# aerospaceresearch/DirectDemod

Measured on AMD Instinct MI355X. Metric: IQ MSamples/s through 255-tap FIR+FM demod, higher is better.
Workload: dtype f32; 1 GPU; C2: 2.4 MS/s complex64 IQ (u8 grid, FM tone + noise), offsetFreq 25 kHz NCO + 255-tap Hamming FIR + FM demod, single chunk, 2^26 samples per GPU, device resident; samples_per_gpu=67108864, ntaps=255, decimation=1, kernel=k_chain_cos1k

## Files before the change

### directdemod_amd/_hip.py

```python
import ctypes as C
import functools
import os
import threading
from fractions import Fraction

import numpy as np

_HERE = os.path.dirname(os.path.abspath(__file__))
LIB_PATH = os.path.join(_HERE, "libdirectdemod_hip.so")
if os.environ.get("DD_LIB_PATH"):
    LIB_PATH = os.path.abspath(os.environ["DD_LIB_PATH"])
    import sys as _sys
    _sys.stderr.write("directdemod_amd: DD_LIB_PATH set, loading %s instead of the product library\n" % LIB_PATH)

DD_OK = 0
DD_ERR_INVALID = -1
DD_ERR_HIP = -2
DD_ERR_NOMEM = -3
DD_ERR_UNSUPPORTED = -4
DD_ERR_NODEVICE = -5
DD_ERR_TIMEOUT = -6

DD_HIST_ZEROS, DD_HIST_ONES, DD_HIST_GIVEN = 0, 1, 2
DD_CHAIN_NCO, DD_CHAIN_FM, DD_CHAIN_U8_INPUT, DD_CHAIN_FORCE_DIRECT, DD_CHAIN_TIGHT = 1, 2, 4, 8, 16
# ... 11 lines not shown
class HipError(RuntimeError):
    pass


_p = C.c_void_p
_i64 = C.c_int64
_u64 = C.c_uint64
_int = C.c_int
_sz = C.c_size_t
_pp = C.POINTER(C.c_void_p)
_pi64 = C.POINTER(C.c_int64)

SIGNATURES = {
    "dd_last_error": (C.c_char_p, []),
    "dd_version": (C.c_char_p, []),
    "dd_device_count": (_int, [C.POINTER(_int)]),
    "dd_set_device": (_int, [_int]),
    "dd_get_device": (_int, [C.POINTER(_int)]),
    "dd_copy_warmup": (_int, []),
    "dd_code_warmup": (_int, []),
    "dd_device_name": (_int, [C.c_char_p, _int]),
    "dd_malloc": (_int, [_pp, _sz]),
    "dd_free": (_int, [_p]),
    "dd_memset": (_int, [_p, _int, _sz, _p]),
    "dd_host_alloc_pinned": (_int, [_pp, _sz]),
    "dd_host_free_pinned": (_int, [_p]),
    "dd_host_register": (_int, [_p, _sz]),
    "dd_host_unregister": (_int, [_p]),
    "dd_debug_fill_lds": (_int, [C.c_uint32, _p]),
    "dd_debug_select_kernel": (_int, [C.c_char_p]),
    "dd_debug_seam": (_int, [_int, _int]),
    "dd_debug_fft1k_plan": (_int, [_i64, _int, _int, _int, _int, C.POINTER(_int)]),
    "dd_debug_cos1k_plan": (_int, [_i64, _int, _int, _int, C.POINTER(_int)]),
    "dd_debug_decimw_plan": (_int, [_i64, _i64, _int, _int, _int, _int, C.POINTER(_i64)]),
    "dd_debug_decimb_lds_check": (_int, [_int, _int, _int, C.POINTER(_i64)]),
    "dd_debug_chain_select": (_int, [C.POINTER(C.c_double), _int, _int, _int, _int, C.c_char_p, C.POINTER(_int)]),
    "dd_debug_cos_fit": (_int, [C.POINTER(C.c_double), _int, C.POINTER(C.c_double), C.POINTER(_int)]),
    "dd_debug_sync_envelope": (_int, [_p, _i64, _int, _int, _p, _p]),
    "dd_memcpy_h2d": (_int, [_p, _p, _sz, _p]),
    "dd_memcpy_d2h": (_int, [_p, _p, _sz, _p]),
    "dd_memcpy_d2d": (_int, [_p, _p, _sz, _p]),
    "dd_stream_create": (_int, [_pp]),
    "dd_stream_destroy": (_int, [_p]),
    "dd_stream_sync": (_int, [_p]),
    "dd_event_create": (_int, [_pp]),
    "dd_event_destroy": (_int, [_p]),
    "dd_event_record": (_int, [_p, _p]),
    "dd_event_elapsed_ms": (_int, [_p, _p, C.POINTER(C.c_float)]),
    "dd_event_sync": (_int, [_p]),
    "dd_stream_wait_event": (_int, [_p, _p]),
    "dd_u8iq_to_c64": (_int, [_p, _p, _i64, _p]),
    "dd_nco_c64": (_int, [_p, _p, _i64, _u64, _i64, _p]),
    "dd_nco_c64_freqs": (_int, [_p, _p, _i64, _p, C.c_double, _i64, _p]),
    "dd_fir_create": (_int, [_pp, C.POINTER(C.c_double), _int]),
    "dd_fir_destroy": (_int, [_p]),
    "dd_fir_reset": (_int, [_p, _int, _p, _p]),
    "dd_fir_reset_hist_f64": (_int, [_p, C.POINTER(C.c_double), _p]),
    "dd_fir_c64": (_int, [_p, _p, _p, _i64, _int, _p]),
    "dd_fir_f64": (_int, [_p, _p, _p, _i64, _int, _p]),
    "dd_filtfilt_f64": (_int, [C.POINTER(C.c_double), _int, _p, _p, _i64, _int, _p]),
    "dd_filtfilt_c64": (_int, [C.POINTER(C.c_double), _int, _p, _p, _i64, _p]),
    "dd_iir_create": (_int, [_pp, C.POINTER(C.c_double), C.POINTER(C.c_double), _int, C.POINTER(C.c_double)]),
    "dd_iir_destroy": (_int, [_p]),
    "dd_iir_f64": (_int, [_p, _p, _p, _i64, _int, _int, _p]),
    "dd_iir_c64": (_int, [_p, _p, _p, _i64, _int, _p]),
    "dd_iir_filtfilt_f64": (_int, [_p, _p, _p, _i64, _int, _p]),
# ... 420 lines not shown
```

### directdemod_amd/csrc/dd_chain.hip

```cpp
#include "dd_chain_tile_kernels.h"
#include "dd_cosfir.h"
#include "dd_fftfir.h"
#include <stdlib.h>
#include <atomic>
#include <mutex>

enum { DD_KSEL_UNREAD = -1, DD_KSEL_AUTO = 0, DD_KSEL_AB = 1, DD_KSEL_FFT1K = 2, DD_KSEL_COS1K = 3, DD_KSEL_DECIMP = 4 };
static std::atomic<int> g_kernel_sel{DD_KSEL_UNREAD};
static int kernel_sel_parse(const char* name) {
    if (!name || !*name || strcmp(name, "auto") == 0) return DD_KSEL_AUTO;
    if (strcmp(name, "ab") == 0) return DD_KSEL_AB;
    if (strcmp(name, "fft1k") == 0) return DD_KSEL_FFT1K;
    if (strcmp(name, "cos1k") == 0) return DD_KSEL_COS1K;
    if (strcmp(name, "decimp") == 0) return DD_KSEL_DECIMP;
    return -2;
}
static int kernel_sel() {
    int c = g_kernel_sel.load(std::memory_order_relaxed);
    if (c == DD_KSEL_UNREAD) {
        c = kernel_sel_parse(getenv("DD_MFMA_KERNEL"));
        if (c < 0) c = DD_KSEL_AUTO;
        g_kernel_sel.store(c, std::memory_order_relaxed);
    }
    return c;
// ... 689 lines not shown
}

extern "C" int dd_chain_reset(dd_chain* c, void* stream) {
    DD_REQUIRE(c, "h");
    c->abs_index = 0;
    if (c->fm) dd_fm_reset(c->fm);
    return dd_fir_reset(c->fir, DD_HIST_ONES, nullptr, stream);
}

static inline int chain_off(const dd_chain* c) {
    return next_off(c->abs_index, 0, c->M);
}

extern "C" int64_t dd_chain_out_count(const dd_chain* c, int64_t n) {
    if (!c || n < 0) return -1;
    return dd_fused_out_count(c->fm, n, c->M, chain_off(c));
}

extern "C" int dd_chain_path(const dd_chain* c) {
    if (!c) return DD_ERR_INVALID;
    const int family = fir_select(c->fir, c->M, c->flags, nullptr);
    return (family == DD_FAMILY_COS1K || family == DD_FAMILY_FFT1K || family == DD_FAMILY_MFMA) ? 1 : 0;
}

extern "C" int dd_fir_last_kernel(const dd_fir* f) {
    if (!f) return DD_ERR_INVALID;
    return f->last_kernel;
}

extern "C" long long dd_fir_launch_count(const dd_fir* f) {
    return f ? f->launches : -1;
}

extern "C" int dd_chain_last_kernel(const dd_chain* c) {
    if (!c) return DD_ERR_INVALID;
    return c->fir->last_kernel;
}

extern "C" int dd_chain_process(dd_chain* c, const void* in, void* out, int64_t n, int64_t* n_out, void* stream) {
    DD_REQUIRE(c && n >= 0, "h/n");
    const DDFusedArgs a = fused_args(in, out, n, c->flags & DD_CHAIN_NCO, c->cyc, c->abs_index, c->M, chain_off(c), c->flags, 1);
    int rc = dd_fused_launch(c->fir, c->fm, a, n_out, dd_stream(stream));
    if (rc == DD_OK) c->abs_index += n;
    return rc;
}

extern "C" int dd_chain_process_chunks(dd_chain* c, const void* in, void* out, const int64_t* bounds_host, int nchunks,
                                       int64_t* n_out_host, void* stream) {
    DD_REQUIRE(c && bounds_host && nchunks >= 0, "arguments");
    const char* in0 = reinterpret_cast<const char*>(in) + (nchunks > 0 ? in_elem_size(c->flags) * (size_t)bounds_host[0] : 0);
    int64_t consumed = 0;
    const int rc = fused_chunks(c->fir, c->fm, in0, out, bounds_host, nchunks, c->flags & DD_CHAIN_NCO, c->cyc, c->abs_index, c->M, chain_off(c),
                                c->flags, n_out_host, &consumed, dd_stream(stream));
    c->abs_index += consumed;
    return rc;
}

extern "C" int dd_chain_seek(dd_chain* c, int64_t abs_index, void* stream) {
    DD_REQUIRE(c && abs_index >= 0, "arguments");
    c->abs_index = abs_index;
    if (c->fm) dd_fm_reset(c->fm);
    return dd_fir_reset(c->fir, abs_index == 0 ? DD_HIST_ONES : DD_HIST_ZEROS, nullptr, stream);
}

extern "C" int dd_chain_prime(dd_chain* c, const void* halo_in, int64_t n_halo, int64_t abs_index, void* stream) {
    DD_REQUIRE(c && n_halo >= 0 && abs_index >= 0, "arguments");
// ... 29 lines not shown
```

### directdemod_amd/csrc/dd_cosfir.h

```cpp
#pragma once
#include "dd_chain_kernels.h"

int dd_cos1k_supported(const double* taps, int K, int M, int flags);
int dd_cos1k_create(void** st, const double* taps, int K);
void dd_cos1k_destroy(void* st);
int dd_cos1k_launch(void* st, const DDChainParams& P, hipStream_t stream);
```

### directdemod_amd/csrc/dd_cosfir.hip

```cpp
#include "dd_chain_kernels.h"
#include "dd_cosfir.h"
#include "dd_cosfit.h"
#include "dd_atan.h"
#include <stdlib.h>

typedef float v2f __attribute__((ext_vector_type(2)));
typedef float v4f __attribute__((ext_vector_type(4)));

#define C1_K 255
#define C1_C1 9.996940573e-01f
#define C1_S1 2.473442728e-02f
#define C1_C2 9.987764162e-01f
#define C1_S2 4.945371992e-02f
#define C1_WC0 9.226918151e-01f
#define C1_WS0 3.855383436e-01f
#define C1_WC1 7.027203712e-01f
#define C1_WS1 7.114661481e-01f
#define C1_WC2 -1.236815966e-02f
#define C1_WS2 9.999235114e-01f
#define C1_WC3 -9.996940573e-01f
#define C1_WS3 -2.473442728e-02f
#define C1_ROW 1024
#define C1_GROUP_BYTES 144
#define C1_BUF_BYTES (64 * C1_GROUP_BYTES)
// ... 60 lines not shown
__device__ __forceinline__ v2f c1_bperm(int addr, v2f v) { return (v2f){c1_bperm(addr, v.x), c1_bperm(addr, v.y)}; }

struct C1St { v2f C, S, R; };

#define C1_ROW_SHR(n) (0x110 + (n))
template <int CTRL>
__device__ __forceinline__ float c1_add_dpp(float r) {
    static_assert(CTRL == 0x111 || CTRL == 0x112 || CTRL == 0x114 || CTRL == 0x118, "dpp control");
    if (CTRL == 0x111) asm("v_add_f32_dpp %0, %0, %0 row_shr:1 row_mask:0xf bank_mask:0xf bound_ctrl:1" : "+v"(r));
    if (CTRL == 0x112) asm("v_add_f32_dpp %0, %0, %0 row_shr:2 row_mask:0xf bank_mask:0xf bound_ctrl:1" : "+v"(r));
    if (CTRL == 0x114) asm("v_add_f32_dpp %0, %0, %0 row_shr:4 row_mask:0xf bank_mask:0xf bound_ctrl:1" : "+v"(r));
    if (CTRL == 0x118) asm("v_add_f32_dpp %0, %0, %0 row_shr:8 row_mask:0xf bank_mask:0xf bound_ctrl:1" : "+v"(r));
    return r;
}
template <int CTRL>
__device__ __forceinline__ void c1_scan_step(C1St& t, float wc, float ws) {
    const v2f Cs = (v2f){c1_dpp0<CTRL>(t.C.x), c1_dpp0<CTRL>(t.C.y)};
    const v2f Ss = (v2f){c1_dpp0<CTRL>(t.S.x), c1_dpp0<CTRL>(t.S.y)};
    t.R = (v2f){c1_add_dpp<CTRL>(t.R.x), c1_add_dpp<CTRL>(t.R.y)};
    t.C = c1_fma(wc, Cs, c1_fma(-ws, Ss, t.C));
    t.S = c1_fma(ws, Cs, c1_fma(wc, Ss, t.S));
}

struct C1Carry {
    C1St W;
    C1St V63;
    v2f y63;
    v2f prow;
    int64_t pend_S;
    int cur;
};

#define C1_NO_PEND ((int64_t)-4611686018427387904LL)
__device__ __forceinline__ void c1_flush_angles(const DDCos1kArgs& A, const char* img, int64_t S, int lane) {
    float* const o = reinterpret_cast<float*>(A.out) + (S - A.s) + 4 * lane;
    const int G = lane >> 2, sw = (G >> 1) & 3;
    v4f v[4];
#pragma unroll
    for (int g = 0; g < 4; ++g) v[g] = *reinterpret_cast<const v4f*>(img + 64 * (16 * g + G) + 16 * ((lane & 3) ^ sw));
#pragma unroll
    for (int g = 0; g < 4; ++g) {
        *reinterpret_cast<v4f*>(o + 256 * g) = v[g];
    }
}

__device__ __forceinline__ void c1_cx_read(const char* img, int lane, v4f (&v)[8]) {
    const char* const rd = img + (lane >> 3) * C1_GROUP_BYTES + 16 * (lane & 7);
#pragma unroll
    for (int j = 0; j < 8; ++j) v[j] = *reinterpret_cast<const v4f*>(rd + 8 * j * C1_GROUP_BYTES);
}
__device__ __forceinline__ void c1_cx_store(const DDCos1kArgs& A, int64_t S, int lane, const v4f (&v)[8]) {
    float2* const o = reinterpret_cast<float2*>(A.out) + S + 2 * lane;
#pragma unroll
    for (int j = 0; j < 8; ++j) __builtin_nontemporal_store(v[j], reinterpret_cast<v4f*>(o + 128 * j));
}

template <bool U8>
__device__ __forceinline__ void c1_issue_loads(const DDCos1kArgs& A, int64_t S, int lane, v4f (&xin)[8]) {
    if (U8) {
        const v4f* p = reinterpret_cast<const v4f*>(reinterpret_cast<const unsigned char*>(A.in) + 2 * (S + 16 * lane));
        xin[0] = __builtin_nontemporal_load(p);
        xin[1] = __builtin_nontemporal_load(p + 1);
    } else {
        const v4f* p = reinterpret_cast<const v4f*>(reinterpret_cast<const float2*>(A.in) + S + 2 * lane);
#pragma unroll
        for (int j = 0; j < 8; ++j) xin[j] = __builtin_nontemporal_load(p + 64 * j);
    }
}

template <bool NCO>
__device__ __forceinline__ v2f c1_row_phasor(const DDCos1kArgs& A, int64_t S, v2f ql) {
    if (!NCO) return (v2f){1.f, 0.f};
    const uint64_t phase64 = (uint64_t)(A.abs0 + S) * A.cyc;
    const uint32_t lo = __builtin_amdgcn_readfirstlane((uint32_t)(phase64 >> (64 - DD_NCO_TBITS - 32)));
#if defined(__HIP_DEVICE_COMPILE__)
    typedef const __attribute__((address_space(4))) float2* c1_const_f2;
    const uint32_t k = __builtin_amdgcn_readfirstlane((uint32_t)(phase64 >> (64 - DD_NCO_TBITS)));
    const float2 Tk = ((c1_const_f2)A.nco_tbl)[k];
#else
    const float2 Tk = make_float2(1.f, 0.f);
#endif
    const float theta = (float)lo * (6.283185307179586f * 5.684341886080802e-14f);
    const float t2 = theta * theta;
    const float cc = fmaf(-0.5f, t2, 1.0f), ss = theta * fmaf(-0.16666667f, t2, 1.0f);
    const v2f pr = (v2f){fmaf(Tk.x, cc, Tk.y * ss), fmaf(Tk.y, cc, -Tk.x * ss)};
    return c1_cmul(pr, ql);
}

template <bool U8, bool NCO, bool EDGE, bool CX>
__device__ __forceinline__ void c1_row(const DDCos1kArgs& A, const DDCos1kLane& lt, const int lane, char* const lds,
                                       const int64_t S, const bool emit, const bool prefetch_next,
                                       v4f (&xin)[8], v4f (&xnext)[8], const v2f ql, C1Carry& cr) {
    const float c = C1_C1, s = C1_S1;
    char* const cur = lds + cr.cur;
    char* const own = cur + lane * C1_GROUP_BYTES;
    v4f pv[8];
    const int64_t cx_pend = CX ? cr.pend_S : C1_NO_PEND;
    if (CX && cx_pend != C1_NO_PEND) { c1_cx_read(cur, lane, pv); cr.pend_S = C1_NO_PEND; }
    const char* const old = lane < 16 ? lds + (C1_BUF_BYTES - cr.cur) + (48 + lane) * C1_GROUP_BYTES : cur + (lane - 16) * C1_GROUP_BYTES;
    v2f xt[16];
    if (EDGE) {
#pragma unroll
        for (int i = 0; i < 16; ++i) {
            const int64_t n = S + 16 * lane + i;
            v2f v = (v2f){0.f, 0.f};
            if (n < 0) {
                const int64_t ti = n + (C1_K - 1);
                if (ti >= 0) v = c1_v2(A.tail_in[ti]);
            } else if (n < A.L) {
                float2 x;
                if (U8) {
                    const uchar2 u = reinterpret_cast<const uchar2*>(A.in)[n];
                    x = make_float2((float)u.x - 127.5f, (float)u.y - 127.5f);
                } else {
                    x = reinterpret_cast<const float2*>(A.in)[n];
                }
                if (NCO) x = dd_cmul(x, dd_phasor((uint64_t)(A.abs0 + n) * A.cyc, A.nco_tbl));
                v = c1_v2(x);
            }
            xt[i] = v;
        }
#pragma unroll
        for (int t = 0; t < 8; ++t) *reinterpret_cast<v4f*>(own + 16 * t) = (v4f){xt[2 * t].x, xt[2 * t].y, xt[2 * t + 1].x, xt[2 * t + 1].y};
    } else {
        const v2f prow = cr.prow;
// ... 28 lines not shown
            v2f pj[8];
            if (NCO) {
                pj[0] = prow;
                pj[1] = c1_cmul(prow, c1_v2(A.q1));
                pj[2] = c1_cmul(prow, c1_v2(A.q2));
                pj[3] = c1_cmul(pj[2], c1_v2(A.q1));
                pj[4] = c1_cmul(prow, c1_v2(A.q4));
                pj[5] = c1_cmul(pj[4], c1_v2(A.q1));
                pj[6] = c1_cmul(pj[4], c1_v2(A.q2));
                pj[7] = c1_cmul(pj[6], c1_v2(A.q1));
            }
            v2f pj1[8], t0[8], t1[8];
            if (NCO) {
                const v2f e1 = c1_v2(A.e1);
#pragma unroll
                for (int j = 0; j < 8; ++j) t0[j] = c1_mul_lo(pj[j], e1);
#pragma unroll
                for (int j = 0; j < 8; ++j) pj1[j] = c1_fma_hi(pj[j], e1, t0[j]);
#pragma unroll
                for (int j = 0; j < 8; ++j) { t0[j] = c1_mul_lo((v2f){xin[j].x, xin[j].y}, pj[j]); t1[j] = c1_mul_lo((v2f){xin[j].z, xin[j].w}, pj1[j]); }
            }
#pragma unroll
            for (int j = 0; j < 8; ++j) {
                v2f x0 = (v2f){xin[j].x, xin[j].y}, x1 = (v2f){xin[j].z, xin[j].w};
                if (NCO) {
                    x0 = c1_fma_hi(x0, pj[j], t0[j]);
                    x1 = c1_fma_hi(x1, pj1[j], t1[j]);
                }
                *reinterpret_cast<v4f*>(wr + 8 * j * C1_GROUP_BYTES) = (v4f){x0.x, x0.y, x1.x, x1.y};
            }
        }
    }
    if (prefetch_next) { c1_issue_loads<U8>(A, S + C1_ROW, lane, xnext); cr.prow = c1_row_phasor<NCO>(A, S + C1_ROW, ql); }
    if (CX) { if (cx_pend != C1_NO_PEND) c1_cx_store(A, cx_pend, lane, pv); }
    else if (cr.pend_S != C1_NO_PEND) { c1_flush_angles(A, lds + (C1_BUF_BYTES - cr.cur), cr.pend_S, lane); cr.pend_S = C1_NO_PEND; }
    if (!EDGE && !U8) {
#pragma unroll
        for (int t = 0; t < 8; ++t) {
            const v4f v = *reinterpret_cast<const v4f*>(own + 16 * t);
            xt[2 * t] = (v2f){v.x, v.y};
            xt[2 * t + 1] = (v2f){v.z, v.w};
        }
    }
    v2f d[16];
    d[0] = *reinterpret_cast<const v2f*>(old + 8);
#pragma unroll
    for (int t = 1; t < 8; ++t) {
        const v4f v = *reinterpret_cast<const v4f*>(old + 16 * t);
        d[2 * t - 1] = (v2f){v.x, v.y};
        d[2 * t] = (v2f){v.z, v.w};
    }
    d[15] = *reinterpret_cast<const v2f*>(lane == 15 ? cur : old + C1_GROUP_BYTES);
    C1St t;
    {
        static constexpr float CW[16] = {1.000000000e+00f, 9.996940573e-01f, 9.987764162e-01f, 9.972476384e-01f, 9.951086592e-01f, 9.923607874e-01f,
                                         9.890057045e-01f, 9.850454633e-01f, 9.804824871e-01f, 9.753195679e-01f, 9.695598648e-01f, 9.632069021e-01f,
                                         9.562645670e-01f, 9.487371075e-01f, 9.406291296e-01f, 9.319455943e-01f};
        static constexpr float SW[16] = {0.000000000e+00f, 2.473442728e-02f, 4.945371992e-02f, 7.414275255e-02f, 9.878641831e-02f, 1.233696381e-01f,
                                         1.478773698e-01f, 1.722946174e-01f, 1.966064405e-01f, 2.207979630e-01f, 2.448543824e-01f, 2.687609789e-01f,
                                         2.925031245e-01f, 3.160662917e-01f, 3.394360625e-01f, 3.625981373e-01f};
        v2f C0 = xt[15], C1 = CW[1] * xt[14], S0 = SW[2] * xt[13], S1 = SW[1] * xt[14], R0 = xt[15] + xt[13], R1 = xt[14];
        C0 = c1_fma(CW[2], xt[13], C0);
#pragma unroll
        for (int i = 12; i >= 0; --i) {
            const int m = 15 - i;
            if (i & 1) { C0 = c1_fma(CW[m], xt[i], C0); S0 = c1_fma(SW[m], xt[i], S0); R0 += xt[i]; }
// ... 108 lines not shown
            for (int g = 0; g < 4; ++g) {
                float worst = -1.0f;
#pragma unroll
                for (int k = 0; k < 4; ++k) worst = fmaxf(worst, fmaf(-0.41421356f, z[4 * g + k].x, fabsf(z[4 * g + k].y)));
                if (__builtin_amdgcn_ballot_w64(worst >= 0.f) == 0) {
#pragma unroll
                    for (int k = 0; k < 4; ++k) ang[4 * g + k] = dd_atan_small(z[4 * g + k].y, z[4 * g + k].x);
                } else {
#pragma unroll
                    for (int k = 0; k < 4; ++k) ang[4 * g + k] = dd_atan2_poly(z[4 * g + k].y, z[4 * g + k].x);
                }
            }
        }
    }
    if (EDGE) {
        float* const o = reinterpret_cast<float*>(A.out) + (S - A.s) + 16 * lane;
#pragma unroll
        for (int i = 0; i < 16; ++i) {
            const int64_t n = S + 16 * lane + i;
            if (n >= A.s && n < A.L) o[i] = ang[i];
        }
        return;
    }
    char* const img = cur;
    {
        const int sw = (lane >> 1) & 3;
#pragma unroll
        for (int t = 0; t < 4; ++t)
            *reinterpret_cast<v4f*>(img + 64 * lane + 16 * (t ^ sw)) = (v4f){ang[4 * t], ang[4 * t + 1], ang[4 * t + 2], ang[4 * t + 3]};
    }
    cr.pend_S = S;
}

template <bool U8>
__device__ __forceinline__ void c1_prime_issue(const DDCos1kArgs& A, int64_t S, int lane, v4f (&xp)[2]) {
    xp[0] = xp[1] = (v4f){0.f, 0.f, 0.f, 0.f};
    if (U8) {
        if (lane >= 48) {
            const v4f* p = reinterpret_cast<const v4f*>(reinterpret_cast<const unsigned char*>(A.in) + 2 * (S + 16 * lane));
            xp[0] = __builtin_nontemporal_load(p);
            xp[1] = __builtin_nontemporal_load(p + 1);
        }
    } else {
        const v4f* p = reinterpret_cast<const v4f*>(reinterpret_cast<const float2*>(A.in) + S + 2 * lane);
        xp[0] = __builtin_nontemporal_load(p + 64 * 6);
        xp[1] = __builtin_nontemporal_load(p + 64 * 7);
    }
}
template <bool U8, bool NCO>
__device__ __forceinline__ void c1_prime_light(const DDCos1kArgs& A, const DDCos1kLane& lt, const int lane, char* const lds, const int64_t S,
                                               const v4f (&xp)[2], const v2f ql, C1Carry& cr) {
    const float c = C1_C1, s = C1_S1;
    char* const cur = lds + cr.cur;
    char* const own = cur + lane * C1_GROUP_BYTES;
    const bool act = lane >= 48;
    const v2f prow = c1_row_phasor<NCO>(A, S, ql);
    v2f xt[16];
#pragma unroll
    for (int i = 0; i < 16; ++i) xt[i] = (v2f){0.f, 0.f};
    if (U8) {
        if (act) {
            unsigned u[8];
#pragma unroll
            for (int t = 0; t < 4; ++t) { u[t] = __float_as_uint(xp[0][t]); u[4 + t] = __float_as_uint(xp[1][t]); }
            v2f p4[4];
            if (NCO) {
                p4[0] = prow;
                p4[1] = c1_cmul(prow, c1_v2(A.e4));
                p4[2] = c1_cmul(prow, c1_v2(A.e8));
                p4[3] = c1_cmul(p4[2], c1_v2(A.e4));
            }
#pragma unroll
            for (int i = 0; i < 16; ++i) {
                const unsigned word = u[i >> 1];
                v2f x = (v2f){(float)((word >> (16 * (i & 1))) & 0xFF) - 127.5f, (float)((word >> (16 * (i & 1) + 8)) & 0xFF) - 127.5f};
                if (NCO) {
                    const v2f pb = p4[i >> 2];
                    x = c1_cmul(x, (i & 3) == 0 ? pb : c1_cmul(pb, c1_v2((i & 3) == 1 ? A.e1 : ((i & 3) == 2 ? A.e2 : A.e3))));
                }
                xt[i] = x;
            }
#pragma unroll
            for (int t = 0; t < 8; ++t) *reinterpret_cast<v4f*>(own + 16 * t) = (v4f){xt[2 * t].x, xt[2 * t].y, xt[2 * t + 1].x, xt[2 * t + 1].y};
        }
    } else {
        char* const wr = cur + (lane >> 3) * C1_GROUP_BYTES + 16 * (lane & 7);
#pragma unroll
        for (int jj = 0; jj < 2; ++jj) {
            const int j = 6 + jj;
// ... 32 lines not shown
            if (i & 1) { C0 = c1_fma(CW[m], xt[i], C0); S0 = c1_fma(SW[m], xt[i], S0); R0 += xt[i]; }
            else { C1 = c1_fma(CW[m], xt[i], C1); S1 = c1_fma(SW[m], xt[i], S1); R1 += xt[i]; }
        }
        t.C = C0 + C1; t.S = S0 + S1; t.R = R0 + R1;
    }
    c1_scan_step<C1_ROW_SHR(1)>(t, C1_WC0, C1_WS0);
    c1_scan_step<C1_ROW_SHR(2)>(t, C1_WC1, C1_WS1);
    c1_scan_step<C1_ROW_SHR(4)>(t, C1_WC2, C1_WS2);
    c1_scan_step<C1_ROW_SHR(8)>(t, C1_WC3, C1_WS3);
    const int back16 = ((lane - 16) & 63) << 2;
    cr.W.C = c1_bperm(back16, t.C);
    cr.W.S = c1_bperm(back16, t.S);
    cr.W.R = c1_bperm(back16, t.R);
    const C1St P63 = {c1_lane63(t.C), c1_lane63(t.S), c1_lane63(t.R)};
    cr.V63.C = c1_fma(-c, e, P63.C);
    cr.V63.S = c1_fma(-s, e, P63.S);
    cr.V63.R = P63.R - e;
    cr.y63 = c1_fma(A.a1 / A.a0, cr.V63.C, cr.V63.R);
    cr.cur = C1_BUF_BYTES - cr.cur;
}

template <bool U8, bool NCO, bool CX>
__global__ void __launch_bounds__(64 * C1_WAVES, 2) k_chain_cos1k(const DDCos1kArgs A) {
    extern __shared__ __attribute__((aligned(16))) char c1_smem[];
    const int lane = threadIdx.x & 63, wave = __builtin_amdgcn_readfirstlane(threadIdx.x >> 6);
    const int gw = blockIdx.x * C1_WAVES + wave;
    const int nrows = A.nrows, nwaves = A.nwaves;
    char* const lds = c1_smem + wave * C1_WAVE_BYTES;
    const DDCos1kLane lt = A.lane_tab[lane];
    v2f ql = (v2f){1.f, 0.f};
    if (NCO) ql = c1_v2(dd_phasor((uint64_t)(U8 ? 16 * lane : 2 * lane) * A.cyc, A.nco_tbl));
    const int R = A.run_rows;
    const int nruns = R > 0 ? (nrows + R - 1) / R : nwaves;
    for (int run = gw; run < nruns; run += nwaves) {
    const int q0 = R > 0 ? run * R : (int)(((int64_t)nrows * gw) / nwaves);
    const int q1 = R > 0 ? (q0 + R < nrows ? q0 + R : nrows) : (int)(((int64_t)nrows * (gw + 1)) / nwaves);
    if (q1 <= q0) continue;
    if (lane < 16) {
#pragma unroll
        for (int t = 0; t < 9; ++t) *reinterpret_cast<v4f*>(lds + C1_BUF_BYTES + (48 + lane) * C1_GROUP_BYTES + 16 * t) = (v4f){0.f, 0.f, 0.f, 0.f};
    }
    C1Carry cr;
    cr.W = cr.V63 = (C1St){(v2f){0.f, 0.f}, (v2f){0.f, 0.f}, (v2f){0.f, 0.f}};
    cr.y63 = (v2f){0.f, 0.f};
    cr.prow = (v2f){1.f, 0.f};
    cr.cur = 0;
    cr.pend_S = C1_NO_PEND;
    auto edge = [&](int q) { const int64_t lo = (int64_t)A.base + (int64_t)C1_ROW * q; return lo < A.s || lo + C1_ROW > A.L || q == nrows - 1; };
    int f0 = q0 - 1;
    const int qfirst = q0 - 1;
    while (f0 < q1 && edge(f0)) ++f0;
    int f1 = f0;
    while (f1 < q1 && !edge(f1)) ++f1;
    v4f xa[8], xb[8];
#pragma unroll
    for (int j = 0; j < 8; ++j) xa[j] = xb[j] = (v4f){0.f, 0.f, 0.f, 0.f};
    for (int q = qfirst; q < f0; ++q)
        c1_row<U8, NCO, true, CX>(A, lt, lane, lds, (int64_t)A.base + (int64_t)C1_ROW * q, q >= q0, false, xa, xb, ql, cr);
    if (f1 > f0) {
        const int64_t S0 = (int64_t)A.base + (int64_t)C1_ROW * f0;
        if (f0 == q0 - 1 && f1 > q0) {
            v4f xp[2];
            c1_prime_issue<U8>(A, S0, lane, xp);
            ++f0;
            c1_issue_loads<U8>(A, S0 + C1_ROW, lane, xa);
            c1_prime_light<U8, NCO>(A, lt, lane, lds, S0, xp, ql, cr);
            cr.prow = c1_row_phasor<NCO>(A, S0 + C1_ROW, ql);
        } else {
            c1_issue_loads<U8>(A, S0, lane, xa);
            cr.prow = c1_row_phasor<NCO>(A, S0, ql);
        }
        for (int q = f0; q < f1; q += 2) {
            const int64_t S = (int64_t)A.base + (int64_t)C1_ROW * q;
            c1_row<U8, NCO, false, CX>(A, lt, lane, lds, S, q >= q0, q + 1 < f1, xa, xb, ql, cr);
            if (q + 1 < f1) c1_row<U8, NCO, false, CX>(A, lt, lane, lds, S + C1_ROW, true, q + 2 < f1, xb, xa, ql, cr);
        }
    }
    if (cr.pend_S != C1_NO_PEND) {
        if (CX) { v4f pv[8]; c1_cx_read(lds + cr.cur, lane, pv); c1_cx_store(A, cr.pend_S, lane, pv); }
        else c1_flush_angles(A, lds + (C1_BUF_BYTES - cr.cur), cr.pend_S, lane);
        cr.pend_S = C1_NO_PEND;
    }
    for (int q = f1; q < q1; ++q)
        c1_row<U8, NCO, true, CX>(A, lt, lane, lds, (int64_t)A.base + (int64_t)C1_ROW * q, q >= q0, false, xa, xb, ql, cr);
    if (q1 == nrows && A.tail_out) {
        for (int i = lane; i < C1_K - 1; i += 64) {
            const int64_t n = A.L - (C1_K - 1) + i;
            float2 v;
            if (n < 0) {
                v = A.tail_in[n + (C1_K - 1)];
            } else {
                float2 x;
                if (U8) {
                    const uchar2 u = reinterpret_cast<const uchar2*>(A.in)[n];
                    x = make_float2((float)u.x - 127.5f, (float)u.y - 127.5f);
                } else {
                    x = reinterpret_cast<const float2*>(A.in)[n];
                }
                v = NCO ? dd_cmul(x, dd_phasor((uint64_t)(A.abs0 + n) * A.cyc, A.nco_tbl)) : x;
            }
            A.tail_out[i] = v;
        }
    }
    }
}

struct DDCos1kState {
    double a0, a1;
    DDCos1kLane* lane_tab;
};

int dd_cos1k_supported(const double* taps, int K, int M, int flags) {
    (void)flags;
    if (M != 1 || K != C1_K) return 0;
    DDCosFit f;
    if (!dd_cos_fit_cached(taps, K, &f)) return 0;
    if (f.Q != 1) return 0;
    return (isfinite(f.a[0]) && isfinite(f.a[1]) && fabs(f.a[0]) >= 1e-3 * fabs(f.a[1]) && f.a[0] != 0.0) ? 1 : 0;
}

int dd_cos1k_create(void** st, const double* taps, int K) {
    if (K != C1_K) return DD_ERR_UNSUPPORTED;
    DDCosFit f;
    if (!dd_cos_fit_cached(taps, K, &f) || f.Q != 1 || !dd_cos1k_supported(taps, K, 1, 0)) return DD_ERR_UNSUPPORTED;
    DDCos1kState* s = new DDCos1kState();
    s->a0 = f.a[0];
    s->a1 = f.a[1];
    s->lane_tab = nullptr;
    DDCos1kLane h[64];
    const long double phi16 = 16.0L * 2.0L * 3.14159265358979323846264338327950288L / (long double)(C1_K - 1);
    for (int l = 0; l < 64; ++l) {
        h[l].b15c = (float)cosl(phi16 * ((l & 15) + 1)); h[l].b15s = (float)sinl(phi16 * ((l & 15) + 1));
    }
    hipError_t e = hipMalloc((void**)&s->lane_tab, sizeof(h));
    if (e == hipSuccess) e = hipMemcpy(s->lane_tab, h, sizeof(h), hipMemcpyHostToDevice);
    if (e != hipSuccess) {
        if (s->lane_tab) (void)hipFree(s->lane_tab);
        delete s;
        dd_set_error("dd_cos1k_create: %s", hipGetErrorString(e));
        return DD_ERR_HIP;
    }
    *st = s;
    return DD_OK;
}

void dd_cos1k_destroy(void* stv) {
    DDCos1kState* s = reinterpret_cast<DDCos1kState*>(stv);
    if (!s) return;
    if (s->lane_tab) (void)hipFree(s->lane_tab);
    delete s;
}

static void cos1k_plan(int64_t L, int s, int out_align_elems, int ncu, int wg_per_cu, int* base, int* nrows, int* grid, int* nwaves) {
    int b = s - out_align_elems;
    while (b > L - 1) b -= 16;
    const int64_t nr = (L - b + C1_ROW - 1) / C1_ROW;
    int g = ncu * (wg_per_cu > 0 ? wg_per_cu : 2);
    if ((int64_t)g * C1_WAVES > nr) g = (int)((nr + C1_WAVES - 1) / C1_WAVES);
    *base = b; *nrows = (int)nr; *grid = g; *nwaves = g * C1_WAVES;
}
extern "C" int dd_debug_cos1k_plan(int64_t L, int s, int out_align_elems, int ncu, int* out) {
    DD_REQUIRE(L >= 1 && (s == 0 || s == 1) && out_align_elems >= 0 && out_align_elems < 16 && ncu >= 1 && out, "arguments");
    cos1k_plan(L, s, out_align_elems, ncu, 2, &out[0], &out[1], &out[2], &out[3]);
    return DD_OK;
}

static const void* cos1k_kernel(bool u8, bool nco, bool cx) {
    static const void* const k[8] = {
        (const void*)k_chain_cos1k<false, false, false>, (const void*)k_chain_cos1k<true, false, false>,
        (const void*)k_chain_cos1k<false, true, false>,  (const void*)k_chain_cos1k<true, true, false>,
        (const void*)k_chain_cos1k<false, false, true>,  (const void*)k_chain_cos1k<true, false, true>,
        (const void*)k_chain_cos1k<false, true, true>,   (const void*)k_chain_cos1k<true, true, true>};
    return k[(u8 ? 1 : 0) | (nco ? 2 : 0) | (cx ? 4 : 0)];
}

int dd_cos1k_launch(void* stv, const DDChainParams& P, hipStream_t stream) {
    DDCos1kState* s = reinterpret_cast<DDCos1kState*>(stv);
    if (P.L < 1) return DD_OK;
    static DDOncePerDevice attr;
    if (attr.need()) {
        for (int i = 0; i < 8; ++i) DD_HIP_CHECK(hipFuncSetAttribute(cos1k_kernel(i & 1, i & 2, i & 4), hipFuncAttributeMaxDynamicSharedMemorySize, C1_LDS_BYTES));
        attr.mark();
    }
    const bool nco = (P.flags & DD_CHAIN_NCO) != 0;
    const long double PI2 = 2.0L * 3.14159265358979323846264338327950288L;
    const long double frac = nco ? (long double)P.cyc / 18446744073709551616.0L : 0.0L;
    DDCos1kArgs A;
    A.in = P.in; A.out = P.out;
    A.tail_in = P.tail_in; A.tail_out = P.tail_out; A.lasty_in = P.lasty_in; A.lasty_out = P.lasty_out;
    A.nco_tbl = P.nco_tbl; A.lane_tab = s->lane_tab;
    A.cyc = P.cyc; A.abs0 = P.abs0; A.L = P.L; A.s = P.s;
    A.a0 = (float)s->a0; A.a1 = (float)s->a1;
    auto ph = [&](int m) { long double p = frac * (long double)m; p -= floorl(p); const long double a = PI2 * p; return make_float2((float)cosl(a), (float)-sinl(a)); };
    A.q1 = ph(128); A.q2 = ph(256); A.q4 = ph(512);
    A.e1 = ph(1); A.e2 = ph(2); A.e3 = ph(3); A.e4 = ph(4); A.e8 = ph(8);
    const bool cx = !(P.flags & DD_CHAIN_FM);
    const int a16 = (int)((reinterpret_cast<uintptr_t>(P.out) >> (cx ? 3 : 2)) & 15);
    int grid;
    cos1k_plan(P.L, P.s, a16, dd_cu_count(), 2, &A.base, &A.nrows, &grid, &A.nwaves);
    A.run_rows = A.nrows >= 16 * A.nwaves ? 8 : 0;
    const bool u8 = (P.flags & DD_CHAIN_U8_INPUT) != 0;
    const dim3 g(grid), b(64 * C1_WAVES);
    void* kargs[1] = {&A};
    DD_HIP_CHECK(hipLaunchKernel(cos1k_kernel(u8, nco, cx), g, b, kargs, C1_LDS_BYTES, stream));
    return DD_OK;
}

int dd_code_touch_cosfir(void) {
    hipFuncAttributes a;
    return hipFuncGetAttributes(&a, (const void*)k_chain_cos1k<false, true, false>) == hipSuccess ? DD_OK : DD_ERR_HIP;
}
```

### include/directdemod_hip_debug.h

```cpp
#ifndef DIRECTDEMOD_HIP_DEBUG_H
#define DIRECTDEMOD_HIP_DEBUG_H

#include <stddef.h>
#include <stdint.h>

#ifdef __cplusplus
extern "C" {
#endif

int  dd_debug_fill_lds(uint32_t pattern, void* stream);
int  dd_debug_select_kernel(const char* name);
int  dd_debug_seam(int withhold_chunk, int spin_log2);
int  dd_debug_fft1k_plan(int64_t L, int s, int out_align_elems, int ncu, int rounds, int* out);
int  dd_debug_cos1k_plan(int64_t L, int s, int out_align_elems, int ncu, int* out);
int  dd_debug_decimw_plan(int64_t abs0, int64_t Ld, int K, int M, int off, int ncu, int64_t* out);
int  dd_debug_decimb_lds_check(int K, int M, int phi, int64_t* out);
#define DD_FAMILY_DENSE 0
#define DD_FAMILY_TILES 1
#define DD_FAMILY_ROWS 2
#define DD_FAMILY_COS1K 3
#define DD_FAMILY_FFT1K 4
#define DD_FAMILY_MFMA 5
int  dd_debug_chain_select(const double* taps_host, int ntaps, int decim, int flags, int in_align_bytes, const char* selector_name, int* family);
int  dd_debug_cos_fit(const double* taps_host, int K, double* a_out, int* Q_out);
int  dd_debug_sync_envelope(const void* X_dev, int64_t L, int nwin, int route, double* env_dev, void* stream);

#ifdef __cplusplus
}
#endif
#endif
```

Before: 485,900 MSamples/s.

## Prefetch next run's start rows during the last interior row of cos1k runs

In the run-scheduled cos1k kernel, a wave that will start another light run now issues the prime and first-row loads (plus row phasors) for that next run while it finishes the final interior row of the current run. This hides the global-load latency at each run boundary, which the loop previously exposed. Debug hooks to override workgroup count and run length, and a host-side plan checker, are added. The cost is extra live registers and more complex control flow that could hurt occupancy. Prefetch only fires for FM output with an even interior row count.

```diff
diff --git a/directdemod_amd/_hip.py b/directdemod_amd/_hip.py
--- a/directdemod_amd/_hip.py
+++ b/directdemod_amd/_hip.py
@@ -67,6 +67,8 @@
     "dd_debug_seam": (_int, [_int, _int]),
     "dd_debug_fft1k_plan": (_int, [_i64, _int, _int, _int, _int, C.POINTER(_int)]),
     "dd_debug_cos1k_plan": (_int, [_i64, _int, _int, _int, C.POINTER(_int)]),
+    "dd_debug_cos1k_runs": (_int, [_p, _int, _int]),
+    "dd_debug_cos1k_run_plan": (_int, [_i64, _int, _int, _int, _int, _int, C.POINTER(_int)]),
     "dd_debug_decimw_plan": (_int, [_i64, _i64, _int, _int, _int, _int, C.POINTER(_i64)]),
     "dd_debug_decimb_lds_check": (_int, [_int, _int, _int, C.POINTER(_i64)]),
     "dd_debug_chain_select": (_int, [C.POINTER(C.c_double), _int, _int, _int, _int, C.c_char_p, C.POINTER(_int)]),
diff --git a/directdemod_amd/csrc/dd_chain.hip b/directdemod_amd/csrc/dd_chain.hip
--- a/directdemod_amd/csrc/dd_chain.hip
+++ b/directdemod_amd/csrc/dd_chain.hip
@@ -745,6 +745,16 @@
     return f ? f->launches : -1;
 }
 
+extern "C" int dd_debug_cos1k_runs(dd_chain* c, int max_workgroups, int run_rows) {
+    DD_REQUIRE(c && c->fir, "chain");
+    void* st = family_state(c->fir, DD_FAMILY_COS1K);
+    if (!st) {
+        dd_set_error("dd_debug_cos1k_runs: this chain's taps have no k_chain_cos1k state");
+        return DD_ERR_UNSUPPORTED;
+    }
+    return dd_cos1k_debug_runs(st, max_workgroups, run_rows);
+}
+
 extern "C" int dd_chain_last_kernel(const dd_chain* c) {
     if (!c) return DD_ERR_INVALID;
     return c->fir->last_kernel;
diff --git a/directdemod_amd/csrc/dd_cosfir.h b/directdemod_amd/csrc/dd_cosfir.h
--- a/directdemod_amd/csrc/dd_cosfir.h
+++ b/directdemod_amd/csrc/dd_cosfir.h
@@ -5,3 +5,4 @@
 int dd_cos1k_create(void** st, const double* taps, int K);
 void dd_cos1k_destroy(void* st);
 int dd_cos1k_launch(void* st, const DDChainParams& P, hipStream_t stream);
+int dd_cos1k_debug_runs(void* st, int max_workgroups, int run_rows);
diff --git a/directdemod_amd/csrc/dd_cosfir.hip b/directdemod_amd/csrc/dd_cosfir.hip
--- a/directdemod_amd/csrc/dd_cosfir.hip
+++ b/directdemod_amd/csrc/dd_cosfir.hip
@@ -116,6 +116,20 @@
 };
 
 #define C1_NO_PEND ((int64_t)-4611686018427387904LL)
+
+struct C1Next {
+    int64_t S;
+    v4f xp[2];
+    v2f prow0, prow1;
+};
+
+__host__ __device__ inline bool c1_edge_row(int base, int s, int64_t L, int nrows, int q) {
+    const int64_t lo = (int64_t)base + (int64_t)C1_ROW * q;
+    return lo < s || lo + C1_ROW > L || q == nrows - 1;
+}
+__host__ __device__ inline bool c1_light_start(int base, int s, int64_t L, int nrows, int q0) {
+    return q0 >= 1 && q0 < nrows && !c1_edge_row(base, s, L, nrows, q0 - 1) && !c1_edge_row(base, s, L, nrows, q0);
+}
 __device__ __forceinline__ void c1_flush_angles(const DDCos1kArgs& A, const char* img, int64_t S, int lane) {
     float* const o = reinterpret_cast<float*>(A.out) + (S - A.s) + 4 * lane;
     const int G = lane >> 2, sw = (G >> 1) & 3;
@@ -171,10 +185,33 @@
     return c1_cmul(pr, ql);
 }
 
+template <bool U8>
+__device__ __forceinline__ void c1_prime_issue(const DDCos1kArgs& A, int64_t S, int lane, v4f (&xp)[2]) {
+    xp[0] = xp[1] = (v4f){0.f, 0.f, 0.f, 0.f};
+    if (U8) {
+        if (lane >= 48) {
+            const v4f* p = reinterpret_cast<const v4f*>(reinterpret_cast<const unsigned char*>(A.in) + 2 * (S + 16 * lane));
+            xp[0] = __builtin_nontemporal_load(p);
+            xp[1] = __builtin_nontemporal_load(p + 1);
+        }
+    } else {
+        const v4f* p = reinterpret_cast<const v4f*>(reinterpret_cast<const float2*>(A.in) + S + 2 * lane);
+        xp[0] = __builtin_nontemporal_load(p + 64 * 6);
+        xp[1] = __builtin_nontemporal_load(p + 64 * 7);
+    }
+}
+template <bool U8, bool NCO>
+__device__ __forceinline__ void c1_run_request(const DDCos1kArgs& A, int lane, v4f (&xfirst)[8], const v2f ql, C1Next& nx) {
+    c1_prime_issue<U8>(A, nx.S, lane, nx.xp);
+    c1_issue_loads<U8>(A, nx.S + C1_ROW, lane, xfirst);
+    nx.prow0 = c1_row_phasor<NCO>(A, nx.S, ql);
+    nx.prow1 = c1_row_phasor<NCO>(A, nx.S + C1_ROW, ql);
+}
+
 template <bool U8, bool NCO, bool EDGE, bool CX>
 __device__ __forceinline__ void c1_row(const DDCos1kArgs& A, const DDCos1kLane& lt, const int lane, char* const lds,
-                                       const int64_t S, const bool emit, const bool prefetch_next,
-                                       v4f (&xin)[8], v4f (&xnext)[8], const v2f ql, C1Carry& cr) {
+                                       const int64_t S, const bool emit, const bool prefetch_next, const bool prefetch_run,
+                                       v4f (&xin)[8], v4f (&xnext)[8], const v2f ql, C1Carry& cr, C1Next& nx) {
     const float c = C1_C1, s = C1_S1;
     char* const cur = lds + cr.cur;
     char* const own = cur + lane * C1_GROUP_BYTES;
@@ -269,6 +306,7 @@
         }
     }
     if (prefetch_next) { c1_issue_loads<U8>(A, S + C1_ROW, lane, xnext); cr.prow = c1_row_phasor<NCO>(A, S + C1_ROW, ql); }
+    else if (prefetch_run) c1_run_request<U8, NCO>(A, lane, xnext, ql, nx);
     if (CX) { if (cx_pend != C1_NO_PEND) c1_cx_store(A, cx_pend, lane, pv); }
     else if (cr.pend_S != C1_NO_PEND) { c1_flush_angles(A, lds + (C1_BUF_BYTES - cr.cur), cr.pend_S, lane); cr.pend_S = C1_NO_PEND; }
     if (!EDGE && !U8) {
@@ -443,29 +481,13 @@
     cr.pend_S = S;
 }
 
-template <bool U8>
-__device__ __forceinline__ void c1_prime_issue(const DDCos1kArgs& A, int64_t S, int lane, v4f (&xp)[2]) {
-    xp[0] = xp[1] = (v4f){0.f, 0.f, 0.f, 0.f};
-    if (U8) {
-        if (lane >= 48) {
-            const v4f* p = reinterpret_cast<const v4f*>(reinterpret_cast<const unsigned char*>(A.in) + 2 * (S + 16 * lane));
-            xp[0] = __builtin_nontemporal_load(p);
-            xp[1] = __builtin_nontemporal_load(p + 1);
-        }
-    } else {
-        const v4f* p = reinterpret_cast<const v4f*>(reinterpret_cast<const float2*>(A.in) + S + 2 * lane);
-        xp[0] = __builtin_nontemporal_load(p + 64 * 6);
-        xp[1] = __builtin_nontemporal_load(p + 64 * 7);
-    }
-}
 template <bool U8, bool NCO>
-__device__ __forceinline__ void c1_prime_light(const DDCos1kArgs& A, const DDCos1kLane& lt, const int lane, char* const lds, const int64_t S,
-                                               const v4f (&xp)[2], const v2f ql, C1Carry& cr) {
+__device__ __forceinline__ void c1_prime_light(const DDCos1kArgs& A, const DDCos1kLane& lt, const int lane, char* const lds,
+                                               const v4f (&xp)[2], const v2f prow, C1Carry& cr) {
     const float c = C1_C1, s = C1_S1;
     char* const cur = lds + cr.cur;
     char* const own = cur + lane * C1_GROUP_BYTES;
     const bool act = lane >= 48;
-    const v2f prow = c1_row_phasor<NCO>(A, S, ql);
     v2f xt[16];
 #pragma unroll
     for (int i = 0; i < 16; ++i) xt[i] = (v2f){0.f, 0.f};
@@ -564,6 +586,10 @@
     if (NCO) ql = c1_v2(dd_phasor((uint64_t)(U8 ? 16 * lane : 2 * lane) * A.cyc, A.nco_tbl));
     const int R = A.run_rows;
     const int nruns = R > 0 ? (nrows + R - 1) / R : nwaves;
+    auto edge = [&](int q) { return c1_edge_row(A.base, A.s, A.L, nrows, q); };
+    v4f xa[8], xb[8];
+    C1Next nx;
+    bool requested = false;
     for (int run = gw; run < nruns; run += nwaves) {
     const int q0 = R > 0 ? run * R : (int)(((int64_t)nrows * gw) / nwaves);
     const int q1 = R > 0 ? (q0 + R < nrows ? q0 + R : nrows) : (int)(((int64_t)nrows * (gw + 1)) / nwaves);
@@ -578,43 +604,52 @@
     cr.prow = (v2f){1.f, 0.f};
     cr.cur = 0;
     cr.pend_S = C1_NO_PEND;
-    auto edge = [&](int q) { const int64_t lo = (int64_t)A.base + (int64_t)C1_ROW * q; return lo < A.s || lo + C1_ROW > A.L || q == nrows - 1; };
+    if (!requested) {
+#pragma unroll
+        for (int j = 0; j < 8; ++j) xa[j] = (v4f){0.f, 0.f, 0.f, 0.f};
+        nx.S = 0;
+        nx.xp[0] = nx.xp[1] = (v4f){0.f, 0.f, 0.f, 0.f};
+        nx.prow0 = nx.prow1 = (v2f){1.f, 0.f};
+    }
+#pragma unroll
+    for (int j = 0; j < 8; ++j) xb[j] = (v4f){0.f, 0.f, 0.f, 0.f};
     int f0 = q0 - 1;
     const int qfirst = q0 - 1;
     while (f0 < q1 && edge(f0)) ++f0;
     int f1 = f0;
     while (f1 < q1 && !edge(f1)) ++f1;
-    v4f xa[8], xb[8];
-#pragma unroll
-    for (int j = 0; j < 8; ++j) xa[j] = xb[j] = (v4f){0.f, 0.f, 0.f, 0.f};
     for (int q = qfirst; q < f0; ++q)
-        c1_row<U8, NCO, true, CX>(A, lt, lane, lds, (int64_t)A.base + (int64_t)C1_ROW * q, q >= q0, false, xa, xb, ql, cr);
+        c1_row<U8, NCO, true, CX>(A, lt, lane, lds, (int64_t)A.base + (int64_t)C1_ROW * q, q >= q0, false, false, xa, xb, ql, cr, nx);
+    bool request = false;
     if (f1 > f0) {
         const int64_t S0 = (int64_t)A.base + (int64_t)C1_ROW * f0;
         if (f0 == q0 - 1 && f1 > q0) {
-            v4f xp[2];
-            c1_prime_issue<U8>(A, S0, lane, xp);
+            if (!requested) { nx.S = S0; c1_run_request<U8, NCO>(A, lane, xa, ql, nx); }
             ++f0;
-            c1_issue_loads<U8>(A, S0 + C1_ROW, lane, xa);
-            c1_prime_light<U8, NCO>(A, lt, lane, lds, S0, xp, ql, cr);
-            cr.prow = c1_row_phasor<NCO>(A, S0 + C1_ROW, ql);
+            c1_prime_light<U8, NCO>(A, lt, lane, lds, nx.xp, nx.prow0, cr);
+            cr.prow = nx.prow1;
         } else {
             c1_issue_loads<U8>(A, S0, lane, xa);
             cr.prow = c1_row_phasor<NCO>(A, S0, ql);
         }
+        if (!CX && R > 0 && run + nwaves < nruns && f1 == q1 && ((f1 - f0) & 1) == 0 && c1_light_start(A.base, A.s, A.L, nrows, (run + nwaves) * R)) {
+            request = true;
+            nx.S = (int64_t)A.base + (int64_t)C1_ROW * ((run + nwaves) * R - 1);
+        }
         for (int q = f0; q < f1; q += 2) {
             const int64_t S = (int64_t)A.base + (int64_t)C1_ROW * q;
-            c1_row<U8, NCO, false, CX>(A, lt, lane, lds, S, q >= q0, q + 1 < f1, xa, xb, ql, cr);
-            if (q + 1 < f1) c1_row<U8, NCO, false, CX>(A, lt, lane, lds, S + C1_ROW, true, q + 2 < f1, xb, xa, ql, cr);
-        }
-    }
+            c1_row<U8, NCO, false, CX>(A, lt, lane, lds, S, q >= q0, q + 1 < f1, false, xa, xb, ql, cr, nx);
+            if (q + 1 < f1) c1_row<U8, NCO, false, CX>(A, lt, lane, lds, S + C1_ROW, true, q + 2 < f1, request && q + 2 >= f1, xb, xa, ql, cr, nx);
+        }
+    }
+    requested = request;
     if (cr.pend_S != C1_NO_PEND) {
         if (CX) { v4f pv[8]; c1_cx_read(lds + cr.cur, lane, pv); c1_cx_store(A, cr.pend_S, lane, pv); }
         else c1_flush_angles(A, lds + (C1_BUF_BYTES - cr.cur), cr.pend_S, lane);
         cr.pend_S = C1_NO_PEND;
     }
     for (int q = f1; q < q1; ++q)
-        c1_row<U8, NCO, true, CX>(A, lt, lane, lds, (int64_t)A.base + (int64_t)C1_ROW * q, q >= q0, false, xa, xb, ql, cr);
+        c1_row<U8, NCO, true, CX>(A, lt, lane, lds, (int64_t)A.base + (int64_t)C1_ROW * q, q >= q0, false, false, xa, xb, ql, cr, nx);
     if (q1 == nrows && A.tail_out) {
         for (int i = lane; i < C1_K - 1; i += 64) {
             const int64_t n = A.L - (C1_K - 1) + i;
@@ -640,6 +675,7 @@
 struct DDCos1kState {
     double a0, a1;
     DDCos1kLane* lane_tab;
+    int dbg_wgs, dbg_run_rows;
 };
 
 int dd_cos1k_supported(const double* taps, int K, int M, int flags) {
@@ -659,6 +695,7 @@
     s->a0 = f.a[0];
     s->a1 = f.a[1];
     s->lane_tab = nullptr;
+    s->dbg_wgs = s->dbg_run_rows = 0;
     DDCos1kLane h[64];
     const long double phi16 = 16.0L * 2.0L * 3.14159265358979323846264338327950288L / (long double)(C1_K - 1);
     for (int l = 0; l < 64; ++l) {
@@ -694,6 +731,66 @@
 extern "C" int dd_debug_cos1k_plan(int64_t L, int s, int out_align_elems, int ncu, int* out) {
     DD_REQUIRE(L >= 1 && (s == 0 || s == 1) && out_align_elems >= 0 && out_align_elems < 16 && ncu >= 1 && out, "arguments");
     cos1k_plan(L, s, out_align_elems, ncu, 2, &out[0], &out[1], &out[2], &out[3]);
+    return DD_OK;
+}
+
+#define C1_RUN_ROWS 8
+static_assert(C1_RUN_ROWS >= 2 && C1_RUN_ROWS % 2 == 0, "an odd run leaves the wrong sample register set free: no run start would be requested ahead");
+static void cos1k_run_map(int nrows, int max_wgs, int run_rows, int* grid, int* nwaves, int* rr) {
+    if (max_wgs > 0) {
+        if (*grid > max_wgs) { *grid = max_wgs; *nwaves = max_wgs * C1_WAVES; }
+        *rr = run_rows;
+        return;
+    }
+    *rr = nrows >= 16 * *nwaves ? C1_RUN_ROWS : 0;
+}
+extern "C" int dd_debug_cos1k_run_plan(int64_t L, int s, int out_align_elems, int ncu, int max_wgs, int run_rows, int* out) {
+    DD_REQUIRE(L >= 1 && (s == 0 || s == 1) && out_align_elems >= 0 && out_align_elems < 16 && ncu >= 1 && max_wgs >= 0 && run_rows >= 0 && out, "arguments");
+    int base, nrows, grid, nwaves, R;
+    cos1k_plan(L, s, out_align_elems, ncu, 2, &base, &nrows, &grid, &nwaves);
+    cos1k_run_map(nrows, max_wgs, run_rows, &grid, &nwaves, &R);
+    const int nruns = R > 0 ? (nrows + R - 1) / R : nwaves;
+    int light = 0, ahead = 0, odd_tail = 0, max_per_wave = 0;
+    for (int gw = 0; gw < nwaves; ++gw) {
+        bool requested = false;
+        int mine = 0;
+        for (int run = gw; run < nruns; run += nwaves) {
+            const int q0 = R > 0 ? run * R : (int)(((int64_t)nrows * gw) / nwaves);
+            const int q1 = R > 0 ? (q0 + R < nrows ? q0 + R : nrows) : (int)(((int64_t)nrows * (gw + 1)) / nwaves);
+            if (q1 <= q0) continue;
+            ++mine;
+            int f0 = q0 - 1;
+            while (f0 < q1 && c1_edge_row(base, s, L, nrows, f0)) ++f0;
+            int f1 = f0;
+            while (f1 < q1 && !c1_edge_row(base, s, L, nrows, f1)) ++f1;
+            bool request = false;
+            if (f1 > f0) {
+                if (f0 == q0 - 1 && f1 > q0) {
+                    DD_REQUIRE(c1_light_start(base, s, L, nrows, q0), "run start predicate");
+                    ++light;
+                    if (requested) ++ahead;
+                    ++f0;
+                } else {
+                    DD_REQUIRE(!requested, "a requested run start must take the light path");
+                }
+                const bool next_light = R > 0 && run + nwaves < nruns && f1 == q1 && c1_light_start(base, s, L, nrows, (run + nwaves) * R);
+                request = next_light && ((f1 - f0) & 1) == 0;
+                if (next_light && !request) ++odd_tail;
+            } else {
+                DD_REQUIRE(!requested, "a requested run start must have interior rows");
+            }
+            requested = request;
+        }
+        if (mine > max_per_wave) max_per_wave = mine;
+    }
+    out[0] = R; out[1] = nruns; out[2] = nwaves; out[3] = light; out[4] = ahead; out[5] = odd_tail; out[6] = max_per_wave; out[7] = nrows;
+    return DD_OK;
+}
+int dd_cos1k_debug_runs(void* stv, int max_wgs, int run_rows) {
+    DDCos1kState* s = reinterpret_cast<DDCos1kState*>(stv);
+    DD_REQUIRE(s && max_wgs >= 0 && run_rows >= 0 && (max_wgs > 0 || run_rows == 0), "max_workgroups >= 1 with run_rows >= 0, or both 0");
+    s->dbg_wgs = max_wgs;
+    s->dbg_run_rows = run_rows;
     return DD_OK;
 }
 
@@ -730,7 +827,7 @@
     const int a16 = (int)((reinterpret_cast<uintptr_t>(P.out) >> (cx ? 3 : 2)) & 15);
     int grid;
     cos1k_plan(P.L, P.s, a16, dd_cu_count(), 2, &A.base, &A.nrows, &grid, &A.nwaves);
-    A.run_rows = A.nrows >= 16 * A.nwaves ? 8 : 0;
+    cos1k_run_map(A.nrows, s->dbg_wgs, s->dbg_run_rows, &grid, &A.nwaves, &A.run_rows);
     const bool u8 = (P.flags & DD_CHAIN_U8_INPUT) != 0;
     const dim3 g(grid), b(64 * C1_WAVES);
     void* kargs[1] = {&A};
diff --git a/include/directdemod_hip_debug.h b/include/directdemod_hip_debug.h
--- a/include/directdemod_hip_debug.h
+++ b/include/directdemod_hip_debug.h
@@ -13,6 +13,9 @@
 int  dd_debug_seam(int withhold_chunk, int spin_log2);
 int  dd_debug_fft1k_plan(int64_t L, int s, int out_align_elems, int ncu, int rounds, int* out);
 int  dd_debug_cos1k_plan(int64_t L, int s, int out_align_elems, int ncu, int* out);
+struct dd_chain;
+int  dd_debug_cos1k_runs(struct dd_chain* chain, int max_workgroups, int run_rows);
+int  dd_debug_cos1k_run_plan(int64_t L, int s, int out_align_elems, int ncu, int max_workgroups, int run_rows, int* out);
 int  dd_debug_decimw_plan(int64_t abs0, int64_t Ld, int K, int M, int off, int ncu, int64_t* out);
 int  dd_debug_decimb_lds_check(int K, int M, int phi, int64_t* out);
 #define DD_FAMILY_DENSE 0
```

Result: slower. 480,000 MSamples/s (-1.2%).
